# paninski-lab/eks

Hardware: AMD Instinct MI355X
Metric: frames*keypoints smoothed/s + achieved HBM GB/s fraction, singlecam 100k x 256 (higher is better)
Workload: dtype f32

## Files before the change

### eks_amd/csrc/eks_diag.hip

```cpp
#include <hip/hip_runtime.h>

#include <cstdlib>

#include "eks_diag_lane.hpp"
#include "eks_internal.hpp"

namespace eks {

struct LaneMap {
  int N, T, nc;
  int nt_log2;
  int ntile;
  int reverse;
};

__device__ __forceinline__ bool lane_coords(const LaneMap& L, int& n, int& j) {
  const int wave = blockIdx.x * (blockDim.x >> 6) + (threadIdx.x >> 6);
  const int lane = threadIdx.x & 63;
  const int tile = wave % L.ntile;
  const int cg = wave / L.ntile;
  const int nt = 1 << L.nt_log2;
  n = tile * nt + (lane & (nt - 1));
  j = cg * (64 >> L.nt_log2) + (lane >> L.nt_log2);
  return n < L.N && j < L.nc;
}

struct DiagWs {
  float *eA, *eb, *eC, *eEta, *eJ;
  float *pm, *pP, *sEta, *sJ;
};

template <int B, bool UNIT>
__global__ __launch_bounds__(256) void diag_summarize_kernel(LaneMap L, DiagModel M, DiagWs W,
                                                            const float* __restrict__ y,
                                                            const float* __restrict__ var) {
  int n, j;
  if (!lane_coords(L, n, j)) return;
  if (L.reverse) j = L.nc - 1 - j;
  const ChainParams<float> p = load_chain_params(M, n);
  const int t0 = j * B;
  const int len = min(B, L.T - t0);
  const Elem<float> e = summarize_chunk<B, UNIT>(y, var, L.N, n, t0, len, p);
  const size_t o = (size_t)j * L.N + n;
  W.eA[o] = e.A;
  W.eb[o] = e.b;
  W.eC[o] = e.C;
  W.eEta[o] = e.eta;
  W.eJ[o] = e.J;
}

template <int B, bool UNIT, int VS_ROW>
__global__ __launch_bounds__(256) void diag_replay_kernel(LaneMap L, DiagModel M, DiagWs W,
                                                         const float* __restrict__ y,
                                                         const float* __restrict__ var,
                                                         float* __restrict__ ms,
                                                         float* __restrict__ Vs) {
  int n, j;
  if (!lane_coords(L, n, j)) return;
  if (L.reverse) j = L.nc - 1 - j;
  const ChainParams<float> p = load_chain_params(M, n);
  const int t0 = j * B;
  const int len = min(B, L.T - t0);
  const size_t o = (size_t)j * L.N + n;
  replay_chunk<B, UNIT, VS_ROW>(y, var, ms, Vs, L.N, n, n % M.D, t0, len, p, W.pm[o], W.pP[o],
                                W.sEta[o], W.sJ[o]);
}

constexpr int kScanCH = 16;
constexpr int kScanCB = 64;

struct ScanWs {
  float *gA, *gb, *gC, *gEta, *gJ;
  float *bm, *bP, *bEta, *bJ;
  int nblk;
};

__device__ __forceinline__ Elem<float> load_elem(const DiagWs& W, size_t o) {
  return Elem<float>{W.eA[o], W.eb[o], W.eC[o], W.eEta[o], W.eJ[o]};
}

struct ScanLds {
  float A[kScanCB][kScanCH + 1], b[kScanCB][kScanCH + 1], C[kScanCB][kScanCH + 1],
      eta[kScanCB][kScanCH + 1], J[kScanCB][kScanCH + 1];
  __device__ __forceinline__ void put(int i, int c, const Elem<float>& e) {
    A[i][c] = e.A; b[i][c] = e.b; C[i][c] = e.C; eta[i][c] = e.eta; J[i][c] = e.J;
  }
  __device__ __forceinline__ Elem<float> get(int i, int c) const {
    return Elem<float>{A[i][c], b[i][c], C[i][c], eta[i][c], J[i][c]};
// ... 61 lines not shown
  }
  float eta = 0.f, J = 0.f;
  const int npass = (S.nblk + 63) / 64;
  for (int pass = npass - 1; pass >= 0; --pass) {
    const int q0 = pass * 64;
    const Elem<float> own = agg(q0 + lane);
    Elem<float> r = own;
#pragma unroll
    for (int off = 1; off < 64; off <<= 1) {
      const Elem<float> dn = shfl_down_elem(r, off);
      if (lane + off < 64) r = elem_combine(r, dn);
    }
    Elem<float> after = shfl_down_elem(r, 1);
    if (lane == 63) after = elem_identity<float>();
    float eq = eta, Jq = J;
    elem_back(after, eq, Jq);
    if (q0 + lane < S.nblk) {
      const size_t o = (size_t)(q0 + lane) * N + n;
      S.bEta[o] = eq;
      S.bJ[o] = Jq;
    }
    const Elem<float> all{__shfl(r.A, 0), __shfl(r.b, 0), __shfl(r.C, 0), __shfl(r.eta, 0), __shfl(r.J, 0)};
    elem_back(all, eta, J);
  }
}

__global__ __launch_bounds__(kScanCH* kScanCB) void diag_scan_local_kernel(int N, int nc, DiagWs W,
                                                                          ScanWs S) {
  __shared__ ScanLds L;
  const int cl = threadIdx.x % kScanCH, i = threadIdx.x / kScanCH;
  const int n = blockIdx.x * kScanCH + cl, j = blockIdx.y * kScanCB + i;
  const bool live = n < N && j < nc;
  L.put(i, cl, live ? load_elem(W, (size_t)j * N + n) : elem_identity<float>());
  __syncthreads();
  const int w = threadIdx.x >> 6, lane = threadIdx.x & 63;
  const Elem<float> own = L.get(lane, w);
  Elem<float> f = own, r = own;
#pragma unroll
  for (int off = 1; off < kScanCB; off <<= 1) {
    const Elem<float> up = shfl_up_elem(f, off), dn = shfl_down_elem(r, off);
    if (lane >= off) f = elem_combine(up, f);
    if (lane + off < kScanCB) r = elem_combine(r, dn);
  }
  Elem<float> excl = shfl_up_elem(f, 1), after = shfl_down_elem(r, 1);
  if (lane == 0) excl = elem_identity<float>();
  if (lane == kScanCB - 1) after = elem_identity<float>();
  const int nw = blockIdx.x * kScanCH + w;
  float m = 0.f, P = 0.f, eta = 0.f, J = 0.f;
  if (nw < N) {
    const size_t ob = (size_t)blockIdx.y * N + nw;
    m = S.bm[ob];
    P = S.bP[ob];
    eta = S.bEta[ob];
    J = S.bJ[ob];
  }
  elem_apply(excl, m, P);
  elem_back(after, eta, J);
  __syncthreads();
  L.A[lane][w] = m;
  L.b[lane][w] = P;
  L.C[lane][w] = eta;
  L.eta[lane][w] = J;
  __syncthreads();
  if (!live) return;
  const size_t o = (size_t)j * N + n;
  W.pm[o] = L.A[i][cl];
  W.pP[o] = L.b[i][cl];
  W.sEta[o] = L.C[i][cl];
  W.sJ[o] = L.eta[i][cl];
}

constexpr int kFW = 4;
static_assert(kFW == 4, "the fused kernels' LDS exchange, the group scan's slot sizes and the measured "
                        "thresholds in diag_smooth() assume four chunks per block");

struct BlockMap {
  int N, T, nc;
  int ntile;
  int ngrp;
  int reverse;
  int tile0;
};

#ifndef EKS_WIN_G
#define EKS_WIN_G 8
#endif
constexpr int kWinG = EKS_WIN_G;
constexpr int kWinH = 2;
constexpr int kWinW = kWinG + 2 * kWinH;
constexpr float kWinTol = 0x1p-30f;
constexpr int kWinDefault = 1;
constexpr int kWinMinT = 32768;
constexpr int kProbeWin = 8;
constexpr int kProbeLen = 64;
static_assert(kWinG % kFW == 0, "the four chunks of an exact-replay block belong to one window group");
static_assert(kWinG >= kWinH, "only the first window group's halo is cut by frame 0");

struct WinWs {
  unsigned char* slow;
  unsigned char* fail;
  int* gate;
  int nwg;
  int nan_bad;
};

struct BufferRows {
  __amdgpu_buffer_rsrc_t ry, rv;
  unsigned voff, row_bytes;
  __device__ __forceinline__ float load_y(int i) const {
    return __builtin_bit_cast(float, __builtin_amdgcn_raw_buffer_load_b32(ry, voff, (unsigned)i * row_bytes, 0));
  }
  __device__ __forceinline__ float load_var(int i) const {
    return __builtin_bit_cast(float, __builtin_amdgcn_raw_buffer_load_b32(rv, voff, (unsigned)i * row_bytes, 0));
  }
};

__device__ __forceinline__ __amdgpu_buffer_rsrc_t rows_rsrc(const float* base) {
  return __builtin_amdgcn_make_buffer_rsrc(const_cast<float*>(base), 0, 0x7FFFFFFF, 0x00020000);
}

constexpr int kAuxNt = 2;

template <int VS_ROW>
struct BufferStore {
  __amdgpu_buffer_rsrc_t rm, rV;
  unsigned voff, row_bytes;
  int d;
  __device__ __forceinline__ void operator()(int i, float m, float P) const {
    constexpr unsigned W = VS_ROW == 0 ? 1 : VS_ROW;
    const unsigned so = (unsigned)i * row_bytes;
    __builtin_amdgcn_raw_buffer_store_b32(__builtin_bit_cast(unsigned, m), rm, voff, so, kAuxNt);
    if constexpr (VS_ROW <= 1) {
      __builtin_amdgcn_raw_buffer_store_b32(__builtin_bit_cast(unsigned, P), rV, voff, so, kAuxNt);
    } else if constexpr (VS_ROW == 2) {
      typedef unsigned u2 __attribute__((ext_vector_type(2)));
      const u2 v = {__builtin_bit_cast(unsigned, d == 0 ? P : 0.0f), __builtin_bit_cast(unsigned, d == 1 ? P : 0.0f)};
      __builtin_amdgcn_raw_buffer_store_b64(v, rV, voff * 2, so * 2, kAuxNt);
    } else {
      typedef unsigned u2 __attribute__((ext_vector_type(2)));
#pragma unroll
      for (unsigned e = 0; e + 1 < W; e += 2) {
        const u2 v = {__builtin_bit_cast(unsigned, (int)e == d ? P : 0.0f),
                      __builtin_bit_cast(unsigned, (int)e + 1 == d ? P : 0.0f)};
        __builtin_amdgcn_raw_buffer_store_b64(v, rV, voff * W + 4 * e, so * W, kAuxNt);
        asm volatile("" ::: "memory");
      }
      if constexpr (W % 2 == 1)
        __builtin_amdgcn_raw_buffer_store_b32(__builtin_bit_cast(unsigned, (int)W - 1 == d ? P : 0.0f), rV,
                                              voff * W + 4 * (W - 1), so * W, kAuxNt);
      asm volatile("" ::: "memory");
    }
  }
};

template <int B, bool UNIT, bool RC>
__global__ __launch_bounds__(64 * kFW) void diag_summarize_blk_kernel(BlockMap L, DiagModel M, DiagWs W,
                                                                     ScanWs S,
                                                                     const float* __restrict__ y,
                                                                     const float* __restrict__ var,
                                                                     const int* __restrict__ gate) {
  __shared__ float sh[5][kFW][64];
  __shared__ int arrived;
  if (gate && gate[L.tile0 + blockIdx.x % L.ntile] == 0) return;
  const int w = __builtin_amdgcn_readfirstlane(threadIdx.x >> 6), lane = threadIdx.x & 63;
  if (threadIdx.x == 0) arrived = 0;
  __syncthreads();
  const int tile = L.tile0 + blockIdx.x % L.ntile;
  int grp = blockIdx.x / L.ntile;
  if (L.reverse) grp = L.ngrp - 1 - grp;
  const int n = tile * 64 + lane, j = grp * kFW + w;
  Elem<float> e = elem_identity<float>();
  if (n < L.N && j < L.nc) {
    const ChainParams<float> p = load_chain_params(M, n);
    const int t0 = j * B, len = min(B, L.T - t0);
    const size_t first = (size_t)t0 * L.N + (size_t)tile * 64;
    const BufferRows rows{rows_rsrc(y + first), rows_rsrc(var + first), (unsigned)lane * 4, (unsigned)L.N * 4};
    float yy[B], rr[B];
    if (len == B) {
      load_rows<B, true>(rows, B, yy, rr);
      e = summarize_loaded<B, UNIT, true>(yy, rr, B, p);
    } else {
      load_rows<B, false>(rows, len, yy, rr);
      e = summarize_loaded<B, UNIT, false>(yy, rr, len, p);
    }
    if constexpr (!RC) {
      const size_t o = (size_t)j * L.N + n;
// ... 97 lines not shown
}

template <int B, bool UNIT, int VS_ROW>
__device__ __forceinline__ void replay_window_block(const BlockMap& L, const DiagModel& M, const WinWs& Wn,
                                                    const float* __restrict__ y, const float* __restrict__ var,
                                                    float* __restrict__ ms, float* __restrict__ Vs) {
  __shared__ float sh[5][kWinW][64];
  __shared__ float shy[64];
  const int w = __builtin_amdgcn_readfirstlane(threadIdx.x >> 6), lane = threadIdx.x & 63;
  const int tile = L.tile0 + blockIdx.x % L.ntile;
  int wg = blockIdx.x / L.ntile;
  if (L.reverse) wg = Wn.nwg - 1 - wg;
  const int n = tile * 64 + lane;
  constexpr int VW = VS_ROW == 0 ? 1 : VS_ROW;
  const bool slow = n >= L.N || (Wn.slow != nullptr && Wn.slow[n] != 0);
  if (__ballot(!slow) == 0) return;
  const int jh0 = wg * kWinG - kWinH;
  const int j = jh0 + w;
  const bool valid = j >= 0 && j < L.nc;
  const bool live = n < L.N && valid;
  ChainParams<float> p{1.f, 1.f, 0.f};
  const int t0 = valid ? j * B : 0;
  const int len = valid ? min(B, L.T - t0) : 0;
  const bool full = len == B;
  const size_t first = (size_t)t0 * L.N + (size_t)tile * 64;
  const BufferRows rows{rows_rsrc(y + first), rows_rsrc(var + first), (unsigned)lane * 4, (unsigned)L.N * 4};
  float v0[B], v1[B];
  Elem<float> own = elem_identity<float>();
  float y0 = 0.f;
  if (live) {
    p = load_chain_params(M, n);
    if (full) {
      load_rows<B, true>(rows, B, v0, v1);
      y0 = v0[0];
      own = summarize_loaded<B, UNIT, true>(v0, v1, B, p);
    } else {
      load_rows<B, false>(rows, len, v0, v1);
      y0 = v0[0];
      own = summarize_loaded<B, UNIT, false>(v0, v1, len, p);
    }
  }
  sh[0][w][lane] = own.A; sh[1][w][lane] = own.b; sh[2][w][lane] = own.C; sh[3][w][lane] = own.eta;
  sh[4][w][lane] = own.J;
  if (w == 0) shy[lane] = y0;
  __syncthreads();
  const int wo = w - kWinH;
  if (wo < 0 || wo >= kWinG || !live) return;
  auto lds_elem = [&](int q) {
    return Elem<float>{sh[0][q][lane], sh[1][q][lane], sh[2][q][lane], sh[3][q][lane], sh[4][q][lane]};
  };
  const bool cut_front = jh0 <= 0, cut_back = (wg + 1) * kWinG + kWinH >= L.nc;
  Elem<float> hf = lds_elem(0), hb = lds_elem(kWinH + kWinG);
#pragma unroll
  for (int q = 1; q < kWinH; ++q) {
    hf = elem_combine(hf, lds_elem(q));
    hb = elem_combine(hb, lds_elem(kWinH + kWinG + q));
  }
  float m, P;
  load_chain_prior(M, n, m, P);
  if (!cut_front) m = UNIT ? shy[lane] : shy[lane] * rcp(p.c);
  const bool good = !slow && fabsf(m) <= 3e38f && (cut_front || fabsf(hf.A) <= kWinTol) &&
                    (cut_back || fabsf(hb.A) <= kWinTol);
  if (!good && !slow && wo == 0 && Wn.fail != nullptr) {
    Wn.fail[(size_t)wg * L.N + n] = 1;
    atomicOr(&Wn.gate[tile], 1);
  }
  elem_apply(hf, m, P);
  for (int q = 0; q < wo; ++q) elem_apply(lds_elem(kWinH + q), m, P);
  if (full) filter_loaded<B, UNIT, true>(v0, v1, B, p, m, P);
  else filter_loaded<B, UNIT, false>(v0, v1, len, p, m, P);
  float eta = 0.f, J = 0.f;
  elem_back(hb, eta, J);
  for (int q = kWinG - 1; q > wo; --q) elem_back(lds_elem(kWinH + q), eta, J);
  fuse_info(m, P, eta, J);
  if (Wn.nan_bad && !good) m = P = __builtin_nanf("");
  const BufferStore<VS_ROW> st{rows_rsrc(ms + first), rows_rsrc(Vs + first * VW), (unsigned)lane * 4,
                               (unsigned)L.N * 4, n % M.D};
  if (good || Wn.nan_bad) {
    if (full) smooth_rows<B, UNIT, true>(v0, v1, B, p, m, P, st);
    else smooth_rows<B, UNIT, false>(v0, v1, len, p, m, P, st);
  }
}

constexpr int kFormElems = 0;
constexpr int kFormRecompute = 1;
constexpr int kFormWindow = 2;

template <int B, bool UNIT, int VS_ROW, int FORM>
__global__ __launch_bounds__(FORM == kFormWindow ? 64 * kWinW : 64 * kFW) void diag_replay_blk_kernel(
    BlockMap L, DiagModel M, DiagWs W, ScanWs S, WinWs Wn, const float* __restrict__ y, const float* __restrict__ var,
    float* __restrict__ ms, float* __restrict__ Vs) {
  if constexpr (FORM == kFormWindow) {
    replay_window_block<B, UNIT, VS_ROW>(L, M, Wn, y, var, ms, Vs);
  } else if constexpr (FORM == kFormRecompute) {
    replay_recompute_block<B, UNIT, VS_ROW, false>(L, M, S, Wn, y, var, ms, Vs);
  } else {
    const int w = __builtin_amdgcn_readfirstlane(threadIdx.x >> 6), lane = threadIdx.x & 63;
    const int tile = L.tile0 + blockIdx.x % L.ntile;
    int grp = blockIdx.x / L.ntile;
    if (L.reverse) grp = L.ngrp - 1 - grp;
    const int n = tile * 64 + lane, j = grp * kFW + w;
    const int j0 = grp * kFW, j1 = min(j0 + kFW, L.nc);
    constexpr int VW = VS_ROW == 0 ? 1 : VS_ROW;
    if (n >= L.N || j >= L.nc) return;
    const ChainParams<float> p = load_chain_params(M, n);
    const int t0 = j * B;
    const int len = min(B, L.T - t0);
    const bool full = len == B;
    const size_t first = (size_t)t0 * L.N + (size_t)tile * 64;
    const BufferRows rows{rows_rsrc(y + first), rows_rsrc(var + first), (unsigned)lane * 4, (unsigned)L.N * 4};
    float v0[B], v1[B];
    if (full) load_rows<B, true>(rows, B, v0, v1);
    else load_rows<B, false>(rows, len, v0, v1);
    Elem<float> ef[kFW - 1];
#pragma unroll
    for (int q = 0; q < kFW - 1; ++q)
      if (j0 + q < j) ef[q] = load_elem(W, (size_t)(j0 + q) * L.N + n);
    const size_t ob = (size_t)grp * L.N + n;
    float m = S.bm[ob], P = S.bP[ob], eta = S.bEta[ob], J = S.bJ[ob];
#pragma unroll
    for (int q = 0; q < kFW - 1; ++q)
      if (j0 + q < j) elem_apply(ef[q], m, P);
    Elem<float> eb[kFW - 1];
#pragma unroll
    for (int q = 0; q < kFW - 1; ++q)
      if (j + 1 + q < j1) eb[q] = load_elem(W, (size_t)(j + 1 + q) * L.N + n);
    if (full) filter_loaded<B, UNIT, true>(v0, v1, B, p, m, P);
    else filter_loaded<B, UNIT, false>(v0, v1, len, p, m, P);
#pragma unroll
    for (int q = kFW - 2; q >= 0; --q)
      if (j + 1 + q < j1) elem_back(eb[q], eta, J);
    fuse_info(m, P, eta, J);
    const BufferStore<VS_ROW> st{rows_rsrc(ms + first), rows_rsrc(Vs + first * VW), (unsigned)lane * 4,
                                 (unsigned)L.N * 4, n % M.D};
    if (full) smooth_rows<B, UNIT, true>(v0, v1, B, p, m, P, st);
    else smooth_rows<B, UNIT, false>(v0, v1, len, p, m, P, st);
  }
}

template <int B, bool UNIT, int VS_ROW>
__global__ __launch_bounds__(64 * kFW) void diag_replay_exact_kernel(BlockMap L, DiagModel M, ScanWs S, WinWs Wn,
                                                                    const float* __restrict__ y,
                                                                    const float* __restrict__ var,
                                                                    float* __restrict__ ms,
                                                                    float* __restrict__ Vs) {
  replay_recompute_block<B, UNIT, VS_ROW, true>(L, M, S, Wn, y, var, ms, Vs);
}

__global__ __launch_bounds__(64 * kProbeWin) void diag_window_probe_kernel(int N, int T, DiagModel M, WinWs Wn,
                                                                          const float* __restrict__ var,
                                                                          int classify) {
  __shared__ int bad[kProbeWin][64];
  const int w = __builtin_amdgcn_readfirstlane(threadIdx.x >> 6), lane = threadIdx.x & 63;
  const int tile = blockIdx.x, n = tile * 64 + lane;
  for (int i = threadIdx.x; i < Wn.nwg * 64; i += 64 * kProbeWin) {
    const int c = tile * 64 + (i & 63);
    if (c < N) Wn.fail[(size_t)(i >> 6) * N + c] = 0;
  }
  int s = 0;
  if (classify && n < N) {
    const ChainParams<float> p = load_chain_params(M, n);
    const int t0 = (int)((long long)w * (T - kProbeLen) / (kProbeWin - 1));
    const float* v = var + (size_t)t0 * N + n;
    float r[kProbeLen];
#pragma unroll
    for (int i = 0; i < kProbeLen; ++i) r[i] = v[(size_t)i * N];
    float A = 1.f, C = 0.f;
#pragma unroll
    for (int i = 0; i < kProbeLen; ++i) {
      const float ri = clip_var(r[i]);
      const float rg = ri * rcp(ri + C * p.c * p.c);
      A = p.times_a(A * rg);
      C = p.times_a2(C * rg) + p.q_s;
    }
    s = !(fabsf(A) <= kWinTol);
// ... 73 lines not shown
#pragma unroll
      for (int i = 0; i < PER; ++i)
        if (b0 + i < q1) e[i] = agg(b0 + i);
    }
#pragma unroll
    for (int i = 0; i < PER; ++i)
      if (b0 + i < q1) {
        const size_t o = (size_t)(b0 + i) * N + n;
        S.bm[o] = m;
        S.bP[o] = P;
        elem_apply(e[i], m, P);
      }
  }
  for (int b1 = q1; b1 > q0; b1 -= PER) {
    const int lo = max(q0, b1 - PER);
    if (!held) {
#pragma unroll
      for (int i = 0; i < PER; ++i)
        if (lo + i < b1) e[i] = agg(lo + i);
    }
#pragma unroll
    for (int i = PER - 1; i >= 0; --i)
      if (lo + i < b1) {
        const size_t o = (size_t)(lo + i) * N + n;
        S.bEta[o] = eta;
        S.bJ[o] = J;
        elem_back(e[i], eta, J);
      }
  }
}

#ifndef EKS_DIAG_CHUNK
#define EKS_DIAG_CHUNK 32
#endif
constexpr int kChunk = EKS_DIAG_CHUNK;

static inline size_t plane_bytes(int nc, int N) { return align_up((size_t)nc * N * sizeof(float), 256); }

static inline size_t win_slow_bytes(int N) { return align_up((size_t)N, 256); }
static inline size_t win_fail_bytes(int nc, int N) { return align_up((size_t)((nc + kWinG - 1) / kWinG) * N, 256); }
static inline size_t win_bytes(int nc, int N) {
  return win_slow_bytes(N) + win_fail_bytes(nc, N) + align_up((size_t)((N + 63) / 64) * sizeof(int), 256);
}

size_t diag_smooth_workspace_bytes(int T, int N) {
  const int nc = (T + kChunk - 1) / kChunk;
  const int nblk = (nc + kFW - 1) / kFW;
  return 9 * plane_bytes(nc, N) + 9 * plane_bytes(nblk, N) + win_bytes(nc, N);
}

static LaneMap make_lane_map(int T, int N, int B) {
  LaneMap L;
  L.N = N;
  L.T = T;
  L.nc = (T + B - 1) / B;
  int nt_log2 = 0;
  while ((1 << nt_log2) < N && nt_log2 < 6) ++nt_log2;
  L.nt_log2 = nt_log2;
  L.ntile = (N + (1 << nt_log2) - 1) >> nt_log2;
  L.reverse = 0;
  return L;
}

template <bool UNIT>
static void launch_replay(int vs_row, dim3 grid, hipStream_t st, const LaneMap& L, const DiagModel& M,
                          const DiagWs& W, const float* y, const float* var, float* ms, float* Vs) {
#define EKS_REPLAY(R)                                                                             \
  case R:                                                                                         \
    hipLaunchKernelGGL((diag_replay_kernel<kChunk, UNIT, R>), grid, dim3(256), 0, st, L, M, W, y, \
                       var, ms, Vs);                                                              \
    break;
  switch (vs_row) {
    EKS_REPLAY(0)
    EKS_REPLAY(1)
    EKS_REPLAY(2)
    EKS_REPLAY(3)
    EKS_REPLAY(4)
    EKS_REPLAY(5)
    EKS_REPLAY(6)
    EKS_REPLAY(7)
    EKS_REPLAY(8)
  }
#undef EKS_REPLAY
}

int diag_smooth(const eks_dims_t& d, const float* y, const float* var, const DiagModel& M,
                float* ms, float* Vs, void* ws, size_t ws_bytes, hipStream_t st) {
  const int T = d.n_frames, D = d.state_dim, N = d.n_keypoints * D;
  const bool vs_diag = d.flags & EKS_FLAG_VS_DIAG;
  if (!vs_diag && D > 8) return EKS_ERR_UNSUPPORTED;
  if (ws_bytes < diag_smooth_workspace_bytes(T, N)) return EKS_ERR_WORKSPACE;
  const LaneMap Lf = make_lane_map(T, N, kChunk);
  const LaneMap& L = Lf;
  const size_t pb = plane_bytes(L.nc, N);
  char* base = static_cast<char*>(ws);
  DiagWs W;
  float** planes[9] = {&W.eA, &W.eb, &W.eC, &W.eEta, &W.eJ, &W.pm, &W.pP, &W.sEta, &W.sJ};
  for (int i = 0; i < 9; ++i) *planes[i] = reinterpret_cast<float*>(base + i * pb);
  const int ngrp_f = (L.nc + kFW - 1) / kFW;
  const bool in_range = (size_t)kChunk * N * (vs_diag ? 1 : D) * sizeof(float) < ((size_t)1 << 31);
  const bool fused = L.nt_log2 == 6 && in_range &&
                     (knob_set(KNOB_SMOOTH_UNFUSED) ? knob_int(KNOB_SMOOTH_UNFUSED, 0) == 0 : ngrp_f <= 1024);
  ScanWs S;
  S.nblk = fused ? (L.nc + kFW - 1) / kFW : (L.nc + kScanCB - 1) / kScanCB;
  const size_t sb = plane_bytes(S.nblk, N);
  float** splanes[9] = {&S.gA, &S.gb, &S.gC, &S.gEta, &S.gJ, &S.bm, &S.bP, &S.bEta, &S.bJ};
  for (int i = 0; i < 9; ++i) *splanes[i] = reinterpret_cast<float*>(base + 9 * pb + i * sb);
  const int vs_row = vs_diag ? 0 : D;
  const bool unit = d.flags & EKS_FLAG_UNIT_AC;
  const int k1_reverse = knob_int(KNOB_SUMMARIZE_REVERSE, 0) == 1 ? 1 : 0;
  const int k3_reverse = knob_set(KNOB_REPLAY_FORWARD) ? (knob_int(KNOB_REPLAY_FORWARD, 0) == 1 ? 0 : 1) : !k1_reverse;
  const int win_mode = knob_int(KNOB_SMOOTH_WINDOW, kWinDefault);
  const int win_min_t = max(kProbeLen, knob_int(KNOB_SMOOTH_WINDOW_MIN_T, kWinMinT));
  const bool windowed = fused && win_mode != 0 && T >= win_min_t;
  WinWs Wn{nullptr, nullptr, nullptr, (L.nc + kWinG - 1) / kWinG, 0};
  if (windowed) {
    char* wb = base + 9 * pb + 9 * sb;
    if (win_mode == 2) {
      Wn.nan_bad = 1;
    } else {
      Wn.slow = reinterpret_cast<unsigned char*>(wb);
      Wn.fail = reinterpret_cast<unsigned char*>(wb + win_slow_bytes(N));
      Wn.gate = reinterpret_cast<int*>(wb + win_slow_bytes(N) + win_fail_bytes(L.nc, N));
    }
  }
  const int* gate = windowed ? Wn.gate : nullptr;
  if (fused) {
    const bool rc_all = knob_set(KNOB_REPLAY_RECOMPUTE) ? knob_int(KNOB_REPLAY_RECOMPUTE, 0) == 1
                                                        : 5 * pb >= ((size_t)16 << 20);
    const int tp = L.ntile;
    for (int tile0 = 0; tile0 < L.ntile; tile0 += tp) {
    const int ntl = min(tp, L.ntile - tile0);
    const int n0 = tile0 * 64, Np = min(N - n0, ntl * 64);
    BlockMap Bm{N, T, L.nc, ntl, S.nblk, k1_reverse, tile0};
    const dim3 bgrid((unsigned)((long)Bm.ntile * Bm.ngrp)), bblock(64 * kFW);
    const bool rc = rc_all || windowed;
#define EKS_K1_BLK(UN)                                                                                  \
  do {                                                                                                  \
    if (rc)                                                                                             \
      hipLaunchKernelGGL((diag_summarize_blk_kernel<kChunk, UN, true>), bgrid, bblock, 0, st, Bm, M, W, \
                         S, y, var, gate);                                                              \
    else                                                                                                \
      hipLaunchKernelGGL((diag_summarize_blk_kernel<kChunk, UN, false>), bgrid, bblock, 0, st, Bm, M,   \
                         W, S, y, var, gate);                                                           \
  } while (0)
#define EKS_K3_BLK(UN, R)                                                                               \
  do {                                                                                                  \
    if (windowed)                                                                                       \
      hipLaunchKernelGGL((diag_replay_exact_kernel<kChunk, UN, R>), bgrid, bblock, 0, st, Bm, M, S, Wn, \
                         y, var, ms, Vs);                                                               \
    else if (rc)                                                                                        \
      hipLaunchKernelGGL((diag_replay_blk_kernel<kChunk, UN, R, kFormRecompute>), bgrid, bblock, 0, st, \
                         Bm, M, W, S, Wn, y, var, ms, Vs);                                              \
    else                                                                                                \
      hipLaunchKernelGGL((diag_replay_blk_kernel<kChunk, UN, R, kFormElems>), bgrid, bblock, 0, st, Bm, \
                         M, W, S, Wn, y, var, ms, Vs);                                                  \
  } while (0)
#define EKS_K3_WIN(UN, R)                                                                               \
  hipLaunchKernelGGL((diag_replay_blk_kernel<kChunk, UN, R, kFormWindow>), wgrid, dim3(64 * kWinW), 0,  \
                     st, Bw, M, W, S, Wn, y, var, ms, Vs)
#define EKS_REPLAY_WIN(R)                                                                              \
  case R:                                                                                              \
    if (unit)                                                                                          \
      EKS_K3_WIN(true, R);                                                                             \
    else                                                                                               \
      EKS_K3_WIN(false, R);                                                                            \
    break;
    if (windowed) {
      if (win_mode != 2) {
        ProfScope ps("diag_window_probe", st);
        hipLaunchKernelGGL(diag_window_probe_kernel, dim3(ntl), dim3(64 * kProbeWin), 0, st, N, T, M, Wn, var,
                           knob_int(KNOB_SMOOTH_WINDOW_PROBE, 1) != 0 ? 1 : 0);
      }
      {
        ProfScope ps("diag_replay", st);
        BlockMap Bw = Bm;
        Bw.reverse = k3_reverse;
        const dim3 wgrid((unsigned)((long)Bw.ntile * Wn.nwg));
        switch (vs_row) {
          EKS_REPLAY_WIN(0)
          EKS_REPLAY_WIN(1)
          EKS_REPLAY_WIN(2)
          EKS_REPLAY_WIN(3)
          EKS_REPLAY_WIN(4)
          EKS_REPLAY_WIN(5)
          EKS_REPLAY_WIN(6)
          EKS_REPLAY_WIN(7)
          EKS_REPLAY_WIN(8)
        }
      }
      if (win_mode == 2) continue;
    }
    {
      ProfScope ps("diag_summarize", st);
      if (unit)
        EKS_K1_BLK(true);
      else
        EKS_K1_BLK(false);
    }
    {
      ProfScope ps("diag_scan", st);
      const bool ch4 = knob_set(KNOB_SCAN_CH) ? knob_int(KNOB_SCAN_CH, 4) == 4 : Np < 2048;
      const bool per8 = (S.nblk + 63) / 64 <= 8;
      const int Ne = n0 + Np;
      if (ch4) {
        if (per8)
          hipLaunchKernelGGL((diag_scan_groups_kernel<8, 4>), dim3((Np + 3) / 4), dim3(256), 0, st, N, n0, Ne, M, S, gate);
        else
          hipLaunchKernelGGL((diag_scan_groups_kernel<16, 4>), dim3((Np + 3) / 4), dim3(256), 0, st, N, n0, Ne, M, S, gate);
      } else {
        if (per8)
          hipLaunchKernelGGL((diag_scan_groups_kernel<8, 16>), dim3((Np + 15) / 16), dim3(1024), 0, st, N, n0, Ne, M, S, gate);
        else
          hipLaunchKernelGGL((diag_scan_groups_kernel<16, 16>), dim3((Np + 15) / 16), dim3(1024), 0, st, N, n0, Ne, M, S, gate);
      }
    }
    ProfScope ps(windowed ? "diag_replay_exact" : "diag_replay", st);
    Bm.reverse = k3_reverse;
#define EKS_REPLAY_BLK(R)                                                                              \
  case R:                                                                                              \
    if (unit)                                                                                          \
      EKS_K3_BLK(true, R);                                                                             \
    else                                                                                               \
      EKS_K3_BLK(false, R);                                                                            \
    break;
    switch (vs_row) {
      EKS_REPLAY_BLK(0)
      EKS_REPLAY_BLK(1)
      EKS_REPLAY_BLK(2)
      EKS_REPLAY_BLK(3)
      EKS_REPLAY_BLK(4)
      EKS_REPLAY_BLK(5)
      EKS_REPLAY_BLK(6)
      EKS_REPLAY_BLK(7)
      EKS_REPLAY_BLK(8)
    }
    }
#undef EKS_REPLAY_BLK
#undef EKS_REPLAY_WIN
#undef EKS_K3_WIN
#undef EKS_K3_BLK
#undef EKS_K1_BLK
    return hip_status(hipGetLastError());
  }

  const int cpw = 64 >> L.nt_log2;
  const long waves = (long)L.ntile * ((L.nc + cpw - 1) / cpw);
  const dim3 grid((unsigned)((waves + 3) / 4));
  {
    ProfScope ps("diag_summarize", st);
    LaneMap L = Lf;
    L.reverse = k1_reverse;
    if (unit)
      hipLaunchKernelGGL((diag_summarize_kernel<kChunk, true>), grid, dim3(256), 0, st, L, M, W, y, var);
    else
      hipLaunchKernelGGL((diag_summarize_kernel<kChunk, false>), grid, dim3(256), 0, st, L, M, W, y, var);
  }
  {
    ProfScope ps("diag_scan", st);
    const dim3 sgrid((N + kScanCH - 1) / kScanCH, S.nblk), sblock(kScanCH * kScanCB);
    hipLaunchKernelGGL(diag_scan_reduce_kernel, sgrid, sblock, 0, st, N, L.nc, W, S);
    hipLaunchKernelGGL(diag_scan_blocks_kernel, dim3((N + 3) / 4), dim3(256), 0, st, N, M, S);
    hipLaunchKernelGGL(diag_scan_local_kernel, sgrid, sblock, 0, st, N, L.nc, W, S);
  }
  {
    ProfScope ps("diag_replay", st);
    LaneMap L = Lf;
    L.reverse = k3_reverse;
    if (unit)
      launch_replay<true>(vs_row, grid, st, L, M, W, y, var, ms, Vs);
    else
      launch_replay<false>(vs_row, grid, st, L, M, W, y, var, ms, Vs);
  }
  return hip_status(hipGetLastError());
}

}

EKS_DEFINE_TOUCH(diag)
```

### eks_amd/csrc/eks_internal.hpp

```cpp
#pragma once
#include <hip/hip_runtime.h>

#include <cstddef>
#include <cstdint>

#include "../../include/eks_hip.h"

namespace eks {

struct DiagModel;

static inline size_t align_up(size_t x, size_t a) { return (x + a - 1) / a * a; }
static inline int hip_status(hipError_t e) { return e == hipSuccess ? EKS_OK : EKS_ERR_HIP_BASE - (int)e; }

__device__ __forceinline__ int xcd_contiguous_block(int b, int nb) {
  const int x = b & 7, i = b >> 3, q = nb >> 3, r = nb & 7;
  return x * q + (x < r ? x : r) + i;
}

enum Knob {
  KNOB_SMOOTH_UNFUSED, KNOB_SUMMARIZE_REVERSE, KNOB_REPLAY_FORWARD, KNOB_REPLAY_RECOMPUTE, KNOB_SCAN_CH,
  KNOB_DENSE_CHUNK, KNOB_NLL_NCL, KNOB_NLL_CHUNK, KNOB_NLL_CHUNK0, KNOB_NLL_WPB,
  KNOB_DENSE_LEGACY, KNOB_NLL_GRAD_UNFUSED, KNOB_NLL_GRAD_CHUNK,
  KNOB_DENSE_TREE_SCAN, KNOB_DENSE_DUAL_GRAD, KNOB_NLL_LEGACY, KNOB_MED_ROWS, KNOB_DW_CHUNK, KNOB_ADAM_PER_ITERATION, KNOB_MED_FINISH_THREADS, KNOB_MED_BRACKET_THREADS, KNOB_NLL_NOLAG, KNOB_NLL_GRAD_TREE, KNOB_ADAM_STREAM, KNOB_ADAM_LAG_RHO_PPM, KNOB_ADAM_LAG_HEAD,
  KNOB_SMOOTH_WINDOW, KNOB_SMOOTH_WINDOW_MIN_T, KNOB_SMOOTH_WINDOW_PROBE, KNOB_COUNT
};
bool knob_set(Knob k);
int knob_int(Knob k, int dflt);

#define EKS_DEFINE_TOUCH(unit)                                                                              \
  namespace eks {                                                                                           \
  __global__ void touch_##unit##_kernel() {}                                                                \
  void touch_##unit() {                                                                                     \
    hipFuncAttributes a;                                                                                    \
    (void)hipFuncGetAttributes(&a, reinterpret_cast<const void*>(touch_##unit##_kernel));                   \
  }                                                                                                         \
  }
void touch_misc();
void touch_diag();
void touch_diag_nll();
void touch_dense();
void touch_dense_wave();
void touch_dense_wide();
void touch_loss();
void touch_loss_ar1();
void touch_multicam();
void touch_lag_adam();

class ProfScope {
 public:
  ProfScope(const char* name, hipStream_t st);
  ~ProfScope();

 private:
  const char* name_;
  hipStream_t st_;
  bool live_;
  hipEvent_t a_, b_;
};

size_t diag_smooth_workspace_bytes(int T, int N);
int diag_smooth(const eks_dims_t& d, const float* y, const float* var, const DiagModel& M,
                float* ms, float* Vs, void* ws, size_t ws_bytes, hipStream_t st);
size_t diag_nll_workspace_bytes(int T, int N, int n_cand);
struct AdamFuse;
int diag_nll(const eks_dims_t& d, const float* y, const double* rconst, const DiagModel& M,
             const double* s_cand, int n_cand, int per_keypoint, double* nll, double* dnll,
             void* ws, size_t ws_bytes, hipStream_t st, const AdamFuse* fuse = nullptr, double* s_out = nullptr,
             int32_t* idx_out = nullptr);
bool diag_nll_grad_tree(int T, int K, int D);
bool diag_nll_adam_persist_ok(int T, int K, int D, int n_blocks);
int diag_nll_adam_persist(const eks_dims_t& d, const float* y, const double* rconst, const DiagModel& M, int n_iters,
                          double* nll, double* dnll, const AdamFuse& F, int32_t* n_active, hipStream_t st);
bool diag_lag_adam_ok(int T, int K, int D, int n_blocks);
size_t diag_lag_adam_workspace_bytes(int T, int N);
int diag_lag_sums(const eks_dims_t& d, const float* y, const double* A, const AdamFuse* F, void* ws, size_t ws_bytes,
                  hipStream_t st);
int diag_lag_adam(const eks_dims_t& d, const float* y, const double* rconst, const DiagModel& M, int n_iters, double* nll,
                  double* dnll, const AdamFuse& F, void* ws, size_t ws_bytes, hipStream_t st);
size_t adam_extra_bytes(int N);
int32_t* nll_ws_tickets(void* ws, int T, int N, int n_cand);
int adam_prepare(int n_blocks, int K, const int32_t* offs, const int32_t* members, int32_t* kp_block,
                 int32_t* counter_a, int32_t* counter_b, hipStream_t st);

bool diag_chain_covers(int T, int N);

size_t diag_sample_workspace_bytes(int T, int N, int n_draws);
int diag_sample(const eks_dims_t& d, const float* y, const float* var, const DiagModel& M, int n_draws, uint64_t seed,
                int first_keypoint, int first_draw, const float* noise, float* ms, float* draws, void* ws,
                size_t ws_bytes, hipStream_t st);
int diag_sample_noise(int T, int N, int D, int n_draws, uint64_t seed, int first_keypoint, int first_draw, float* noise,
                      hipStream_t st);
struct DenseModel;
size_t dense_sample_workspace_bytes(int T, int K, int D, int O, int n_draws);
int dense_sample(const eks_dims_t& d, const float* y, const float* var, const DenseModel& M, int n_draws, uint64_t seed,
                 int first_keypoint, int first_draw, const float* noise, float* ms, float* draws, void* ws,
                 size_t ws_bytes, hipStream_t st);
int dense_sample_noise(int T, int K, int W, int n_draws, uint64_t seed, int first_keypoint, int first_draw, float* noise,
                       hipStream_t st);

struct DenseModel {
  const double *m0, *S0, *A, *C, *Q, *s;
};
size_t diag_increments_workspace_bytes(int T, int N);
int diag_increments(const eks_dims_t& d, const float* y, const float* var, const DiagModel& M, float* ms, float* Vs,
                    float* lag1, float* dmean, float* dV, void* ws, size_t ws_bytes, hipStream_t st);
size_t dense_increments_workspace_bytes(int T, int K, int D, int O);
int dense_increments(const eks_dims_t& d, const float* y, const float* var, const DenseModel& M, float* ms, float* Vs,
// ... 141 lines not shown
```

### eks_amd/csrc/eks_profile.hip

```cpp
#include <hip/hip_runtime.h>

#include <cstdlib>
#include <cstring>
#include <mutex>
#include <vector>

#include "eks_internal.hpp"

namespace eks {

namespace {
struct KnobTable {
  bool set[KNOB_COUNT];
  int val[KNOB_COUNT];
  KnobTable() { load(); }
  int load() {
    static const char* const names[KNOB_COUNT] = {
        "EKS_SMOOTH_UNFUSED", "EKS_SUMMARIZE_REVERSE", "EKS_REPLAY_FORWARD", "EKS_REPLAY_RECOMPUTE", "EKS_SCAN_CH",
        "EKS_DENSE_CHUNK", "EKS_NLL_NCL", "EKS_NLL_CHUNK", "EKS_NLL_CHUNK0", "EKS_NLL_WPB",
        "EKS_DENSE_LEGACY", "EKS_NLL_GRAD_UNFUSED",
        "EKS_NLL_GRAD_CHUNK", "EKS_DENSE_TREE_SCAN", "EKS_DENSE_DUAL_GRAD", "EKS_NLL_LEGACY", "EKS_MED_ROWS", "EKS_DW_CHUNK", "EKS_ADAM_PER_ITERATION", "EKS_MED_FINISH_THREADS", "EKS_MED_BRACKET_THREADS", "EKS_NLL_NOLAG", "EKS_NLL_GRAD_TREE", "EKS_ADAM_STREAM", "EKS_ADAM_LAG_RHO_PPM", "EKS_ADAM_LAG_HEAD",
        "EKS_SMOOTH_WINDOW", "EKS_SMOOTH_WINDOW_MIN_T", "EKS_SMOOTH_WINDOW_PROBE"};
    int n = 0;
    for (int i = 0; i < KNOB_COUNT; ++i) {
      const char* v = getenv(names[i]);
      set[i] = v != nullptr;
      val[i] = v ? atoi(v) : 0;
      n += set[i];
    }
    return n;
  }
};
KnobTable& knob_table() {
  static KnobTable t;
  return t;
}
}

bool knob_set(Knob k) { return knob_table().set[k]; }
int knob_int(Knob k, int dflt) { return knob_table().set[k] ? knob_table().val[k] : dflt; }

struct ProfEntry {
  const char* name;
  hipEvent_t a, b;
};
static int g_prof_level = 0;
static std::vector<ProfEntry> g_prof;
static std::vector<hipEvent_t> g_pool;
static std::mutex g_prof_mu;

static hipEvent_t take_event() {
  std::lock_guard<std::mutex> lk(g_prof_mu);
  if (!g_pool.empty()) {
    hipEvent_t e = g_pool.back();
    g_pool.pop_back();
    return e;
  }
  hipEvent_t e;
  hipEventCreate(&e);
  return e;
}

static bool scope_live(const char* name) {
  if (g_prof_level == 1) return true;
  if (g_prof_level != 2) return false;
  const size_t n = strlen(name);
  return (n >= 7 && strcmp(name + n - 7, "_replay") == 0) || strcmp(name, "diag_nll_summarize") == 0;
}

ProfScope::ProfScope(const char* name, hipStream_t st) : name_(name), st_(st), live_(scope_live(name)) {
  if (!live_) return;
  a_ = take_event();
  b_ = take_event();
  hipEventRecord(a_, st_);
}
ProfScope::~ProfScope() {
  if (!live_) return;
  hipEventRecord(b_, st_);
  std::lock_guard<std::mutex> lk(g_prof_mu);
  g_prof.push_back({name_, a_, b_});
}

}

extern "C" {

int eks_knobs_reload(void) { return eks::knob_table().load(); }

int eks_profile_enable(int on) {
  eks::g_prof_level = on < 0 ? 0 : on > 2 ? 1 : on;
  return EKS_OK;
}

int eks_profile_drain(char* names, size_t names_bytes, float* ms, int32_t max_n) {
  std::lock_guard<std::mutex> lk(eks::g_prof_mu);
  int n = 0;
  size_t off = 0;
  for (auto& e : eks::g_prof) {
    hipEventSynchronize(e.b);
    float t = 0.f;
    hipEventElapsedTime(&t, e.a, e.b);
    eks::g_pool.push_back(e.a);
    eks::g_pool.push_back(e.b);
    const size_t len = strlen(e.name) + 1;
    if (n < max_n && names && ms && off + len <= names_bytes) {
// ... 11 lines not shown
```

Measured before the change: 55.72 billion.

## Walk consecutive window groups per block to reuse halo chunk summaries

Adds a walking form of the windowed replay kernel. Each block now steps through a run of consecutive window groups and keeps chunk summaries and standing y values in an LDS ring, so halo chunks that overlap with the next group are not reloaded and re-summarized. The run length comes from a cost model over CU count and grid size. This cuts redundant HBM reads and summarize work on halos, at the cost of fewer blocks, a per-step __syncthreads, and serialization along each run.

```diff
diff --git a/eks_amd/csrc/eks_diag.hip b/eks_amd/csrc/eks_diag.hip
--- a/eks_amd/csrc/eks_diag.hip
+++ b/eks_amd/csrc/eks_diag.hip
@@ -4,6 +4,7 @@
 
 #include "eks_diag_lane.hpp"
 #include "eks_internal.hpp"
+#include "eks_win_walk.hpp"
 
 namespace eks {
 
@@ -231,12 +232,6 @@
   int tile0;
 };
 
-#ifndef EKS_WIN_G
-#define EKS_WIN_G 8
-#endif
-constexpr int kWinG = EKS_WIN_G;
-constexpr int kWinH = 2;
-constexpr int kWinW = kWinG + 2 * kWinH;
 constexpr float kWinTol = 0x1p-30f;
 constexpr int kWinDefault = 1;
 constexpr int kWinMinT = 32768;
@@ -251,6 +246,7 @@
   int* gate;
   int nwg;
   int nan_bad;
+  int run_len;
 };
 
 struct BufferRows {
@@ -514,15 +510,115 @@
   }
 }
 
+template <int B, bool UNIT, int VS_ROW>
+__device__ __forceinline__ void replay_walk_block(const BlockMap& L, const DiagModel& M, const WinWs& Wn,
+                                                  const float* __restrict__ y, const float* __restrict__ var,
+                                                  float* __restrict__ ms, float* __restrict__ Vs) {
+  __shared__ float sh[5][kWalkRing][64];
+  __shared__ float shy[kWalkStand][64];
+  const int w = __builtin_amdgcn_readfirstlane(threadIdx.x >> 6), lane = threadIdx.x & 63;
+  const int tile = L.tile0 + blockIdx.x % L.ntile;
+  const int run_len = Wn.run_len;
+  int run = blockIdx.x / L.ntile;
+  if (L.reverse) run = (Wn.nwg + run_len - 1) / run_len - 1 - run;
+  const int n = tile * 64 + lane;
+  constexpr int VW = VS_ROW == 0 ? 1 : VS_ROW;
+  const bool slow = n >= L.N || (Wn.slow != nullptr && Wn.slow[n] != 0);
+  if (__ballot(!slow) == 0) return;
+  ChainParams<float> p{1.f, 1.f, 0.f};
+  float m0 = 0.f, P0 = 0.f;
+  if (n < L.N) {
+    p = load_chain_params(M, n);
+    load_chain_prior(M, n, m0, P0);
+  }
+  const int d = n % M.D;
+  float v0[B], v1[B];
+  const int g0 = run * run_len, g1 = min(g0 + run_len, Wn.nwg);
+  for (int g = g0; g < g1; ++g) {
+    const int base = walk_base(g);
+    const int off = walk_off(g, w);
+    const int j = base + off;
+    const bool valid = j >= 0 && j < L.nc;
+    const bool live = n < L.N && valid;
+    const int t0 = valid ? j * B : 0;
+    const int len = valid ? min(B, L.T - t0) : 0;
+    const bool full = len == B;
+    const size_t first = (size_t)t0 * L.N + (size_t)tile * 64;
+    if (walk_loads(off, g == g0)) {
+      Elem<float> own = elem_identity<float>();
+      float y0 = 0.f;
+      if (live) {
+        const BufferRows rows{rows_rsrc(y + first), rows_rsrc(var + first), (unsigned)lane * 4, (unsigned)L.N * 4};
+        if (full) {
+          load_rows<B, true>(rows, B, v0, v1);
+          y0 = v0[0];
+          own = summarize_loaded<B, UNIT, true>(v0, v1, B, p);
+        } else {
+          load_rows<B, false>(rows, len, v0, v1);
+          y0 = v0[0];
+          own = summarize_loaded<B, UNIT, false>(v0, v1, len, p);
+        }
+      }
+      const int slot = walk_elem_slot(j);
+      sh[0][slot][lane] = own.A; sh[1][slot][lane] = own.b; sh[2][slot][lane] = own.C; sh[3][slot][lane] = own.eta;
+      sh[4][slot][lane] = own.J;
+      if (walk_saves_stand(j)) shy[walk_stand_slot(j)][lane] = y0;
+    }
+    __syncthreads();
+    if (!walk_replays(off) || !live) continue;
+    const int wo = off - kWinH;
+    auto lds_elem = [&](int jj) {
+      const int q = walk_elem_slot(jj);
+      return Elem<float>{sh[0][q][lane], sh[1][q][lane], sh[2][q][lane], sh[3][q][lane], sh[4][q][lane]};
+    };
+    const bool cut_front = base <= 0, cut_back = (g + 1) * kWinG + kWinH >= L.nc;
+    Elem<float> hf = lds_elem(base), hb = lds_elem(base + kWinH + kWinG);
+#pragma unroll
+    for (int q = 1; q < kWinH; ++q) {
+      hf = elem_combine(hf, lds_elem(base + q));
+      hb = elem_combine(hb, lds_elem(base + kWinH + kWinG + q));
+    }
+    float m = m0, P = P0;
+    if (!cut_front) {
+      const float ys = shy[walk_stand_slot(base)][lane];
+      m = UNIT ? ys : ys * rcp(p.c);
+    }
+    const bool good = !slow && fabsf(m) <= 3e38f && (cut_front || fabsf(hf.A) <= kWinTol) &&
+                      (cut_back || fabsf(hb.A) <= kWinTol);
+    if (!good && !slow && wo == 0 && Wn.fail != nullptr) {
+      Wn.fail[(size_t)g * L.N + n] = 1;
+      atomicOr(&Wn.gate[tile], 1);
+    }
+    elem_apply(hf, m, P);
+    for (int q = 0; q < wo; ++q) elem_apply(lds_elem(base + kWinH + q), m, P);
+    if (full) filter_loaded<B, UNIT, true>(v0, v1, B, p, m, P);
+    else filter_loaded<B, UNIT, false>(v0, v1, len, p, m, P);
+    float eta = 0.f, J = 0.f;
+    elem_back(hb, eta, J);
+    for (int q = kWinG - 1; q > wo; --q) elem_back(lds_elem(base + kWinH + q), eta, J);
+    fuse_info(m, P, eta, J);
+    if (Wn.nan_bad && !good) m = P = __builtin_nanf("");
+    const BufferStore<VS_ROW> st{rows_rsrc(ms + first), rows_rsrc(Vs + first * VW), (unsigned)lane * 4,
+                                 (unsigned)L.N * 4, d};
+    if (good || Wn.nan_bad) {
+      if (full) smooth_rows<B, UNIT, true>(v0, v1, B, p, m, P, st);
+      else smooth_rows<B, UNIT, false>(v0, v1, len, p, m, P, st);
+    }
+  }
+}
+
 constexpr int kFormElems = 0;
 constexpr int kFormRecompute = 1;
 constexpr int kFormWindow = 2;
+constexpr int kFormWalk = 3;
 
 template <int B, bool UNIT, int VS_ROW, int FORM>
-__global__ __launch_bounds__(FORM == kFormWindow ? 64 * kWinW : 64 * kFW) void diag_replay_blk_kernel(
+__global__ __launch_bounds__(FORM >= kFormWindow ? 64 * kWinW : 64 * kFW) void diag_replay_blk_kernel(
     BlockMap L, DiagModel M, DiagWs W, ScanWs S, WinWs Wn, const float* __restrict__ y, const float* __restrict__ var,
     float* __restrict__ ms, float* __restrict__ Vs) {
-  if constexpr (FORM == kFormWindow) {
+  if constexpr (FORM == kFormWalk) {
+    replay_walk_block<B, UNIT, VS_ROW>(L, M, Wn, y, var, ms, Vs);
+  } else if constexpr (FORM == kFormWindow) {
     replay_window_block<B, UNIT, VS_ROW>(L, M, Wn, y, var, ms, Vs);
   } else if constexpr (FORM == kFormRecompute) {
     replay_recompute_block<B, UNIT, VS_ROW, false>(L, M, S, Wn, y, var, ms, Vs);
@@ -762,6 +858,32 @@
     EKS_REPLAY(8)
   }
 #undef EKS_REPLAY
+}
+
+constexpr int kWalkDefault = 1;
+constexpr int kWalkMinRun = 2;
+
+static int device_cu_count() {
+  static const int n = [] {
+    int dev = 0, c = 0;
+    if (hipGetDevice(&dev) != hipSuccess ||
+        hipDeviceGetAttribute(&c, hipDeviceAttributeMultiprocessorCount, dev) != hipSuccess || c <= 0)
+      c = 256;
+    return c;
+  }();
+  return n;
+}
+
+static int walk_run(int ntile, int nwg) {
+  if (knob_int(KNOB_SMOOTH_WINDOW_WALK, kWalkDefault) == 0) return 0;
+  if (knob_set(KNOB_SMOOTH_WINDOW_RUN)) return min(max(knob_int(KNOB_SMOOTH_WINDOW_RUN, 1), 1), nwg);
+  thread_local int c_ntile = 0, c_nwg = 0, c_run = 0;
+  if (ntile != c_ntile || nwg != c_nwg) {
+    c_run = walk_run_length(ntile, nwg, device_cu_count());
+    c_ntile = ntile;
+    c_nwg = nwg;
+  }
+  return c_run >= kWalkMinRun ? c_run : 0;
 }
 
 int diag_smooth(const eks_dims_t& d, const float* y, const float* var, const DiagModel& M,
@@ -793,7 +915,7 @@
   const int win_mode = knob_int(KNOB_SMOOTH_WINDOW, kWinDefault);
   const int win_min_t = max(kProbeLen, knob_int(KNOB_SMOOTH_WINDOW_MIN_T, kWinMinT));
   const bool windowed = fused && win_mode != 0 && T >= win_min_t;
-  WinWs Wn{nullptr, nullptr, nullptr, (L.nc + kWinG - 1) / kWinG, 0};
+  WinWs Wn{nullptr, nullptr, nullptr, (L.nc + kWinG - 1) / kWinG, 0, 0};
   if (windowed) {
     char* wb = base + 9 * pb + 9 * sb;
     if (win_mode == 2) {
@@ -839,9 +961,17 @@
 #define EKS_K3_WIN(UN, R)                                                                               \
   hipLaunchKernelGGL((diag_replay_blk_kernel<kChunk, UN, R, kFormWindow>), wgrid, dim3(64 * kWinW), 0,  \
                      st, Bw, M, W, S, Wn, y, var, ms, Vs)
+#define EKS_K3_WALK(UN, R)                                                                             \
+  hipLaunchKernelGGL((diag_replay_blk_kernel<kChunk, UN, R, kFormWalk>), wgrid, dim3(64 * kWinW), 0,    \
+                     st, Bw, M, W, S, Ww, y, var, ms, Vs)
 #define EKS_REPLAY_WIN(R)                                                                              \
   case R:                                                                                              \
-    if (unit)                                                                                          \
+    if (run_len > 0) {                                                                                 \
+      if (unit)                                                                                        \
+        EKS_K3_WALK(true, R);                                                                          \
+      else                                                                                             \
+        EKS_K3_WALK(false, R);                                                                         \
+    } else if (unit)                                                                                   \
       EKS_K3_WIN(true, R);                                                                             \
     else                                                                                               \
       EKS_K3_WIN(false, R);                                                                            \
@@ -856,7 +986,10 @@
         ProfScope ps("diag_replay", st);
         BlockMap Bw = Bm;
         Bw.reverse = k3_reverse;
-        const dim3 wgrid((unsigned)((long)Bw.ntile * Wn.nwg));
+        const int run_len = walk_run(Bw.ntile, Wn.nwg);
+        WinWs Ww = Wn;
+        Ww.run_len = run_len;
+        const dim3 wgrid((unsigned)((long)Bw.ntile * (run_len > 0 ? (Wn.nwg + run_len - 1) / run_len : Wn.nwg)));
         switch (vs_row) {
           EKS_REPLAY_WIN(0)
           EKS_REPLAY_WIN(1)
@@ -919,6 +1052,7 @@
 #undef EKS_REPLAY_BLK
 #undef EKS_REPLAY_WIN
 #undef EKS_K3_WIN
+#undef EKS_K3_WALK
 #undef EKS_K3_BLK
 #undef EKS_K1_BLK
     return hip_status(hipGetLastError());
diff --git a/eks_amd/csrc/eks_internal.hpp b/eks_amd/csrc/eks_internal.hpp
--- a/eks_amd/csrc/eks_internal.hpp
+++ b/eks_amd/csrc/eks_internal.hpp
@@ -23,7 +23,8 @@
   KNOB_DENSE_CHUNK, KNOB_NLL_NCL, KNOB_NLL_CHUNK, KNOB_NLL_CHUNK0, KNOB_NLL_WPB,
   KNOB_DENSE_LEGACY, KNOB_NLL_GRAD_UNFUSED, KNOB_NLL_GRAD_CHUNK,
   KNOB_DENSE_TREE_SCAN, KNOB_DENSE_DUAL_GRAD, KNOB_NLL_LEGACY, KNOB_MED_ROWS, KNOB_DW_CHUNK, KNOB_ADAM_PER_ITERATION, KNOB_MED_FINISH_THREADS, KNOB_MED_BRACKET_THREADS, KNOB_NLL_NOLAG, KNOB_NLL_GRAD_TREE, KNOB_ADAM_STREAM, KNOB_ADAM_LAG_RHO_PPM, KNOB_ADAM_LAG_HEAD,
-  KNOB_SMOOTH_WINDOW, KNOB_SMOOTH_WINDOW_MIN_T, KNOB_SMOOTH_WINDOW_PROBE, KNOB_COUNT
+  KNOB_SMOOTH_WINDOW, KNOB_SMOOTH_WINDOW_MIN_T, KNOB_SMOOTH_WINDOW_PROBE,
+  KNOB_SMOOTH_WINDOW_WALK, KNOB_SMOOTH_WINDOW_RUN, KNOB_COUNT
 };
 bool knob_set(Knob k);
 int knob_int(Knob k, int dflt);
diff --git a/eks_amd/csrc/eks_profile.hip b/eks_amd/csrc/eks_profile.hip
--- a/eks_amd/csrc/eks_profile.hip
+++ b/eks_amd/csrc/eks_profile.hip
@@ -20,7 +20,8 @@
         "EKS_DENSE_CHUNK", "EKS_NLL_NCL", "EKS_NLL_CHUNK", "EKS_NLL_CHUNK0", "EKS_NLL_WPB",
         "EKS_DENSE_LEGACY", "EKS_NLL_GRAD_UNFUSED",
         "EKS_NLL_GRAD_CHUNK", "EKS_DENSE_TREE_SCAN", "EKS_DENSE_DUAL_GRAD", "EKS_NLL_LEGACY", "EKS_MED_ROWS", "EKS_DW_CHUNK", "EKS_ADAM_PER_ITERATION", "EKS_MED_FINISH_THREADS", "EKS_MED_BRACKET_THREADS", "EKS_NLL_NOLAG", "EKS_NLL_GRAD_TREE", "EKS_ADAM_STREAM", "EKS_ADAM_LAG_RHO_PPM", "EKS_ADAM_LAG_HEAD",
-        "EKS_SMOOTH_WINDOW", "EKS_SMOOTH_WINDOW_MIN_T", "EKS_SMOOTH_WINDOW_PROBE"};
+        "EKS_SMOOTH_WINDOW", "EKS_SMOOTH_WINDOW_MIN_T", "EKS_SMOOTH_WINDOW_PROBE",
+        "EKS_SMOOTH_WINDOW_WALK", "EKS_SMOOTH_WINDOW_RUN"};
     int n = 0;
     for (int i = 0; i < KNOB_COUNT; ++i) {
       const char* v = getenv(names[i]);
diff --git a/eks_amd/csrc/eks_win_walk.hpp b/eks_amd/csrc/eks_win_walk.hpp
--- /dev/null
+++ b/eks_amd/csrc/eks_win_walk.hpp
@@ -0,0 +1,43 @@
+#pragma once
+
+namespace eks {
+
+#ifndef EKS_WIN_G
+#define EKS_WIN_G 8
+#endif
+constexpr int kWinG = EKS_WIN_G;
+constexpr int kWinH = 2;
+constexpr int kWinW = kWinG + 2 * kWinH;
+static_assert(kWinG >= 2 * kWinH, "the carried chunks of a step and the chunks whose elements the next step's front "
+                                  "halo needs are different own chunks");
+
+constexpr int kWalkRing = 2 * kWinW;
+constexpr int kWalkStand = 3;
+
+constexpr int walk_base(int g) { return g * kWinG - kWinH; }
+constexpr int walk_wave(int j) { return (j + kWinW) % kWinW; }
+constexpr int walk_off(int g, int w) { return (w + kWinW - walk_wave(walk_base(g))) % kWinW; }
+constexpr int walk_chunk(int g, int w) { return walk_base(g) + walk_off(g, w); }
+constexpr bool walk_loads(int off, bool first_step) { return first_step || off >= 2 * kWinH; }
+constexpr bool walk_replays(int off) { return off >= kWinH && off < kWinH + kWinG; }
+constexpr bool walk_keeps(int off) { return off >= kWinH + kWinG; }
+constexpr int walk_elem_slot(int j) { return (j + kWalkRing) % kWalkRing; }
+constexpr bool walk_saves_stand(int j) { return (j + kWinH) % kWinG == 0; }
+constexpr int walk_stand_slot(int j) { return ((j + kWinH) / kWinG) % kWalkStand; }
+
+constexpr int kWalkRunEnd = 1;
+constexpr int walk_run_length(int ntile, int nwg, int ncu) {
+  long best = -1;
+  int br = 1;
+  for (int r = 1; r <= nwg; ++r) {
+    const long blocks = (long)ntile * ((nwg + r - 1) / r);
+    const long cost = ((blocks + ncu - 1) / ncu) * (r + kWalkRunEnd);
+    if (best < 0 || cost < best) {
+      best = cost;
+      br = r;
+    }
+  }
+  return br;
+}
+
+}
```

Result: faster. 56.48 billion, median of 6 (+1.4%).
